# NVIDIA/audio-flamingo

Measured on AMD Instinct MI355X. Metric: audio-sec/s + decoder tokens/s, AF3-7B bf16 train, higher is better.
Workload: dtype bf16; 1 GPU; AF3 (AF-Whisper 32L + Qwen2.5-7B 28L, MLP projector) bf16 train step fwd+bwd+AdamW, 30 s clips, S=1024; micro_batch_per_gpu=8, global_batch=8, seq_len=1024, parallelism=dp1, activation_checkpointing=False

## Files before the change

### audio-flamingo_amd/csrc/gemm.hip

```cpp
#include "gemm_common.h"
#include <vector>
#include <mutex>

namespace {

constexpr int BM = 128, BN = 128, BK = 64;
constexpr int ROWB = BK * 2;
constexpr int STAGE_BYTES = (BM + BN) * ROWB;
constexpr int NSTAGE = 2;

__global__ __launch_bounds__(256, 2) void gemm_nt_bf16_k128(GemmArgs p) {
    extern __shared__ __attribute__((aligned(16))) char smem[];
    const int tid = threadIdx.x;
    const int lane = tid & 63;
    const int wave = __builtin_amdgcn_readfirstlane(tid >> 6);
    const int wm = wave >> 1, wn = wave & 1;
    const int hi = lane >> 5, l31 = lane & 31;

    int tm, tn;
    gemm_tile_of_block(p, tm, tn);
    const int m0 = tm * BM, n0 = tn * BN;

    const bf16* a_src[4];
    const bf16* b_src[4];
// ... 82 lines not shown
    const int lane = threadIdx.x & 63, wave = threadIdx.x >> 6;
    const int n0 = (blockIdx.x * 4 + wave) * R;
    if (n0 >= p.N) return;
    const int kb_all = (p.K + 511) >> 9;
    const int kb0 = (int)((int64_t)kb_all * blockIdx.y / p.splits), kb1 = (int)((int64_t)kb_all * (blockIdx.y + 1) / p.splits);
    float acc[R][MB];
#pragma unroll
    for (int r = 0; r < R; ++r)
#pragma unroll
        for (int m = 0; m < MB; ++m) acc[r][m] = 0.f;
    const bf16* wrow[R];
#pragma unroll
    for (int r = 0; r < R; ++r) wrow[r] = p.B + (int64_t)min(n0 + r, p.N - 1) * p.ldb;
    for (int kb = kb0; kb < kb1; ++kb) {
        const int k = (kb << 9) + lane * 8;
        if (k < p.K) {
            bf16x8 wv[R], xv[MB];
#pragma unroll
            for (int r = 0; r < R; ++r) wv[r] = __builtin_nontemporal_load((const bf16x8*)(wrow[r] + k));
#pragma unroll
            for (int m = 0; m < MB; ++m) xv[m] = *(const bf16x8*)(p.A + (int64_t)min(m, p.M - 1) * p.lda + k);
#pragma unroll
            for (int r = 0; r < R; ++r)
#pragma unroll
                for (int m = 0; m < MB; ++m)
#pragma unroll
                    for (int e = 0; e < 4; ++e) {
                        const bf16x2 a = {wv[r][2 * e], wv[r][2 * e + 1]}, b = {xv[m][2 * e], xv[m][2 * e + 1]};
                        acc[r][m] = __builtin_amdgcn_fdot2_f32_bf16(a, b, acc[r][m], false);
                    }
        }
    }
    constexpr int V = R * MB;
    static_assert((V & (V - 1)) == 0 && V <= 64, "R*MB must be a power of two <= 64");
    float* v = &acc[0][0];
    int n = V;
#pragma unroll
    for (int sft = 5; sft >= 0; --sft) {
        const int st = 1 << sft;
        const bool up = (lane >> sft) & 1;
        if (n > 1) {
            const int h = n >> 1;
#pragma unroll
            for (int i = 0; i < V / 2; ++i)
                if (i < h) {
                    const float lo = v[i], hi_ = v[i + h];
                    v[i] = (up ? hi_ : lo) + __shfl_xor(up ? lo : hi_, st, 64);
                }
            n = h;
        } else {
            v[0] += __shfl_xor(v[0], st, 64);
        }
    }
    constexpr int LOGV = V == 64 ? 6 : V == 32 ? 5 : V == 16 ? 4 : V == 8 ? 3 : V == 4 ? 2 : V == 2 ? 1 : 0;
    const int idx = lane >> (6 - LOGV);
    const int r = idx / MB, m = idx % MB;
    if ((lane & ((64 >> LOGV) - 1)) == 0 && n0 + r < p.N && m < p.M) p.ws[((int64_t)blockIdx.y * p.M + m) * p.N + n0 + r] = v[0];
}

__global__ __launch_bounds__(256) void gemm_splitk_reduce_kernel(GemmArgs p) {
    const int n4 = p.N >> 2;
    const int64_t total = (int64_t)p.M * n4;
    for (int64_t t = (int64_t)blockIdx.x * blockDim.x + threadIdx.x; t < total; t += (int64_t)gridDim.x * blockDim.x) {
        const int m = (int)(t / n4), n = (int)(t % n4) * 4;
        const float* src = p.ws + (int64_t)m * p.N + n;
        f32x4 acc = *(const f32x4*)src;
        for (int sp = 1; sp < p.splits; ++sp) {
            const f32x4 x = *(const f32x4*)(src + (int64_t)sp * p.M * p.N);
#pragma unroll
            for (int e = 0; e < 4; ++e) acc[e] += x[e];
        }
        float v[4] = {acc[0], acc[1], acc[2], acc[3]};
        gemm_epilogue_store4(p, m, n, v);
    }
}

struct ProfState {
    std::mutex mu;
    bool on = false;
    std::vector<hipEvent_t> pool;
    size_t used = 0;
    double flops = 0.0;
    int64_t launches = 0;
    struct Rec { int M, N, K, variant; };
    std::vector<Rec> recs;
};
ProfState g_prof;
int g_variant = 0;
[[maybe_unused]] int g_256_impl = 2;
int g_gm = 0;
int g_wide = 1;
int g_mfma = 0;

constexpr int mfma_shapes(int form) { return form == 0 ? AFK_MFMA_SHAPES_NT : form == 1 ? AFK_MFMA_SHAPES_NN : AFK_MFMA_SHAPES_TN; }
constexpr int AFK_MFMA_RULE_NT = 16, AFK_MFMA_RULE_NN = 32, AFK_MFMA_RULE_TN = 32;
int gemm_mfma_of(int form) {
    static const int env = [] {
        const char* e = getenv("AFK_GEMM_MFMA");
        return (e && e[0] >= '0' && e[0] <= '2' && !e[1]) ? e[0] - '0' : 0;
    }();
    const int sel = g_mfma ? g_mfma : env;
    if (sel == 1) return 32;
    if (sel == 2) return 16;
    return form == 0 ? AFK_MFMA_RULE_NT : form == 1 ? AFK_MFMA_RULE_NN : AFK_MFMA_RULE_TN;
}

hipEvent_t prof_next_event() {
    if (g_prof.used == g_prof.pool.size()) {
        hipEvent_t e;
        hipEventCreate(&e);
        g_prof.pool.push_back(e);
    }
    return g_prof.pool[g_prof.used++];
}

}

extern "C" int afk_gemm_set_variant(int v) {
    const int gm = (v >> 8) & 255, base = v & 15;
#ifdef AFK_PROBES
    AFK_REQUIRE(base >= 0 && base <= 14, "afk_gemm_set_variant: 14 = persistent tile loop with the next tile's prologue issued ahead of the epilogue stores (round-4 probe), 13 = 256x256 ping-pong as a persistent tile loop, 0 auto, 1 = 128x128, 2 = 256x256 8-wave ping-pong, 3 = 256x256 4-wave (4, 5: its timing probes), 6 = 256x256 8-wave free-running BK=64 (7, 8, 9: probes), 10 = 8-wave free-running BK=32 ring-10 (11: probe)");
#else
    AFK_REQUIRE(base >= 0 && base <= 2, "afk_gemm_set_variant: variant %d is a probe / rejected schedule; this libafk.so was built without -DAFK_PROBES (make PROBES=1)", base);
    AFK_REQUIRE((gm & 0xc0) == 0, "afk_gemm_set_variant: gm bits 6 / 7 are timing probes (wrong results); this libafk.so was built without -DAFK_PROBES");
#endif
    g_gm = gm;
    g_wide = (v & 16) ? 0 : 1;
    g_variant = base;
    return AFK_OK;
}

extern "C" int afk_gemm_set_mfma(int v) {
    AFK_REQUIRE(v >= 0 && v <= 2, "afk_gemm_set_mfma: %d (0 = dispatch rule, 1 = 32x32x16, 2 = 16x16x32)", v);
    constexpr int any = AFK_MFMA_SHAPES_NT | AFK_MFMA_SHAPES_NN | AFK_MFMA_SHAPES_TN;
    AFK_REQUIRE(v == 0 || (any >> (v - 1)) & 1, "afk_gemm_set_mfma: no 256x256 kernel of this libafk.so carries the %s shape; build with make PROBES=1",
                v == 1 ? "32x32x16" : "16x16x32");
    g_mfma = v;
    return AFK_OK;
}
extern "C" int afk_gemm_mfma_shapes(int form) { return form >= 0 && form <= 2 ? mfma_shapes(form) : 0; }

extern "C" int afk_prof_enable(int on) {
    std::lock_guard<std::mutex> lk(g_prof.mu);
    g_prof.on = on != 0;
    return AFK_OK;
}

extern "C" int afk_prof_reset(void) {
    std::lock_guard<std::mutex> lk(g_prof.mu);
    g_prof.used = 0;
    g_prof.flops = 0.0;
    g_prof.launches = 0;
    g_prof.recs.clear();
    return AFK_OK;
}

extern "C" int afk_prof_collect(double* total_ms, double* total_flops, int64_t* launches) {
    std::lock_guard<std::mutex> lk(g_prof.mu);
    double ms = 0.0;
    for (size_t i = 0; i + 1 < g_prof.used; i += 2) {
        if (hipEventSynchronize(g_prof.pool[i + 1]) != hipSuccess)
            return afk_set_error(AFK_ERR_LAUNCH, "afk_prof_collect: event sync failed");
        float t = 0.f;
        if (hipEventElapsedTime(&t, g_prof.pool[i], g_prof.pool[i + 1]) != hipSuccess)
            return afk_set_error(AFK_ERR_LAUNCH, "afk_prof_collect: elapsed failed");
        ms += t;
    }
    if (total_ms) *total_ms = ms;
    if (total_flops) *total_flops = g_prof.flops;
    if (launches) *launches = g_prof.launches;
    return AFK_OK;
}

struct RopeEpi { const void *cos_t, *sin_t; const int* pos; int S, cols; const void *cos_lanes, *sin_lanes; };

static int gemm_impl(int trans_a, int trans_b, const void* A, int64_t lda, const void* B, int64_t ldb, void* C, int64_t ldc,
                     int M, int N, int K, const void* bias, const void* residual, int64_t ldr,
                     int res_mod, void* preact_out, float alpha, int flags, void* stream, int splits = 1, void* workspace = nullptr,
                     const RopeEpi* rope = nullptr) {
    AFK_REQUIRE(splits >= 1 && splits <= 64 && (splits == 1 || workspace), "afk_gemm_*_splitk: 1..64 splits, workspace required");
    AFK_REQUIRE(((flags & AFK_GEMM_ROPE) != 0) == (rope != nullptr), "afk_gemm: AFK_GEMM_ROPE belongs to afk_gemm_nt_bf16_rope");
    AFK_REQUIRE(splits == 1 || splits <= (K + BK - 1) / BK, "afk_gemm_*_splitk: more splits than K tiles");
    const bool gemv = workspace != nullptr && M <= AFK_GEMV_MAX_M && !trans_a && !trans_b;
    AFK_REQUIRE(!gemv || splits <= (K + 511) / 512, "afk_gemm_nt_bf16_splitk: M <= 16 streams K in blocks of 512: at most ceil(K/512) splits");
    AFK_REQUIRE(A && B && C, "afk_gemm_nt_bf16: null operand");
    AFK_REQUIRE(M > 0 && N > 0 && K > 0, "afk_gemm_nt_bf16: bad shape %d %d %d", M, N, K);
    AFK_REQUIRE(!trans_a || trans_b, "afk_gemm_bf16: A^T with k-contiguous B is not implemented (NT, NN, TN are)");
    AFK_REQUIRE(trans_a || K % BK == 0, "afk_gemm_nt_bf16: K=%d must be a multiple of %d (pad the operand)", K, BK);
    AFK_REQUIRE(!trans_b || (N % 8 == 0 && N >= 8), "afk_gemm_bf16: N=%d must be a multiple of 8 for a reduction-major B", N);
    AFK_REQUIRE(!trans_a || (M % 8 == 0 && M >= 8), "afk_gemm_bf16: M=%d must be a multiple of 8 for a reduction-major A", M);
    AFK_REQUIRE(N % 4 == 0, "afk_gemm_nt_bf16: N=%d must be a multiple of 4", N);
    AFK_REQUIRE(lda % 8 == 0 && ldb % 8 == 0 && ldc % 4 == 0, "afk_gemm_nt_bf16: leading dims must keep 16-B (A,B) / 8-B (C) alignment");
    AFK_REQUIRE(!(flags & AFK_GEMM_BIAS) || bias, "afk_gemm_nt_bf16: BIAS flag without bias");
    AFK_REQUIRE(!(flags & AFK_GEMM_RESIDUAL) || (residual && ldr % 4 == 0), "afk_gemm_nt_bf16: RESIDUAL flag without residual");
    AFK_REQUIRE(!(flags & AFK_GEMM_SWIGLU_FWD) || (flags == AFK_GEMM_SWIGLU_FWD && !trans_a && !trans_b && preact_out && N % 256 == 0 && splits == 1 &&
                                                     ldc % 8 == 0 && (uintptr_t)C % 16 == 0 && (uintptr_t)preact_out % 16 == 0),
                "afk_gemm_nt_bf16: SWIGLU_FWD needs the NT form, preact_out, N = 2I with I %% 128 == 0 and no other flag");
    AFK_REQUIRE(!(flags & AFK_GEMM_SWIGLU_BWD) || (residual && ldr % 4 == 0 && ldc >= 2 * (int64_t)N && flags == AFK_GEMM_SWIGLU_BWD && splits == 1),
                "afk_gemm: SWIGLU_BWD needs the gate|up tensor as `residual`, a [M, 2N] output and no other epilogue flag");
    AFK_REQUIRE(((uintptr_t)A % 16 == 0) && ((uintptr_t)B % 16 == 0) && ((uintptr_t)C % 8 == 0), "afk_gemm_nt_bf16: misaligned pointer");
    GemmArgs p;
    p.A = (const bf16*)A;
    p.B = (const bf16*)B;
    p.C = C;
    p.C2 = preact_out;
    p.bias = (const bf16*)bias;
    p.R = (const bf16*)residual;
    p.lda = lda;
    p.ldb = ldb;
    p.ldc = ldc;
    p.ldr = ldr;
    p.M = M;
    p.N = N;
    p.K = K;
    p.flags = flags;
    p.res_mod = res_mod;
    p.alpha = alpha;
    p.gm = g_gm;
    p.splits = splits;
    p.ws = (float*)workspace;
    p.rope_cos = rope ? (const bf16*)rope->cos_t : nullptr;
    p.rope_sin = rope ? (const bf16*)rope->sin_t : nullptr;
    p.rope_pos = rope ? rope->pos : nullptr;
    p.rope_S = rope ? rope->S : 1;
    p.rope_cols = rope ? rope->cols : 0;
    const bool lanes_ok = rope && rope->cos_lanes && rope->sin_lanes && !rope->pos && rope->S % 32 == 0;
    p.rope_cos_lanes = lanes_ok ? (const bf16*)rope->cos_lanes : nullptr;
    p.rope_sin_lanes = lanes_ok ? (const bf16*)rope->sin_lanes : nullptr;
    {
        const bool f32 = (flags & AFK_GEMM_OUT_F32) != 0;
        bool w = N % 8 == 0 && ldc % 8 == 0 && (uintptr_t)C % (f32 ? 32 : 16) == 0;
        if (flags & AFK_GEMM_BIAS) w = w && (uintptr_t)bias % 16 == 0;
        if (flags & (AFK_GEMM_RESIDUAL | AFK_GEMM_SWIGLU_BWD)) w = w && ldr % 8 == 0 && (uintptr_t)residual % 16 == 0;
        if (preact_out) w = w && (uintptr_t)preact_out % 16 == 0;
        p.wide = w && g_wide ? 1 : 0;
    }
    const int64_t tiles256 = afk_cdiv(M, 256) * afk_cdiv(N, 256);
    const bool use256 = !gemv && (trans_b || (flags & AFK_GEMM_SWIGLU_FWD) || (splits == 1 && (g_variant >= 2 || (g_variant == 0 && tiles256 >= 192))));
    if (rope && (!use256 || !p.wide || trans_a || trans_b || splits != 1))
        return afk_set_error(AFK_ERR_UNSUPPORTED, "afk_gemm_nt_bf16_rope: needs the 256 x 256 NT kernel (>= 192 tiles) in its 16-byte epilogue form; use "
                                                  "afk_gemm_nt_bf16 + afk_rope_inplace for this shape");
#ifdef AFK_PROBES
    static const int env_impl = [] {
        const char* e = getenv("AFK_GEMM256");
        return (e && e[0] == 'p' && e[1] == 'e') ? 13 : (e && e[0] == 'p') ? 2 : (e && e[0] == 'w') ? 3 : (e && e[0] == 'f') ? 10 : 0;
    }();
    const int impl256 = (flags & (AFK_GEMM_SWIGLU_FWD | AFK_GEMM_ROPE)) ? 2 : g_variant >= 2 ? g_variant : (env_impl ? env_impl : g_256_impl);
    const bool w4 = use256 && !trans_b && impl256 >= 3 && impl256 <= 9;
    const bool f8 = use256 && !trans_b && impl256 >= 10 && impl256 <= 12;
    const bool persist = use256 && !trans_b && impl256 == 13;
    const bool persist_q = use256 && !trans_b && impl256 == 14;
#endif
    if ((flags & AFK_GEMM_SWIGLU_FWD) && !p.wide)
        return afk_set_error(AFK_ERR_UNSUPPORTED, "afk_gemm_nt_bf16: SWIGLU_FWD needs the 16-byte epilogue form (aligned C / preact_out, ldc %% 8 == 0, "
                                                  "afk_gemm_set_variant bit 4 clear)");
    p.ntm = (int)afk_cdiv(M, use256 ? 256 : BM);
    p.ntn = (int)afk_cdiv(N, use256 ? 256 : BN);
    static bool attr_set = false;
    if (!attr_set) {
        hipFuncSetAttribute((const void*)gemm_nt_bf16_k128, hipFuncAttributeMaxDynamicSharedMemorySize, NSTAGE * STAGE_BYTES);
        attr_set = true;
    }
    hipStream_t st = (hipStream_t)stream;
    const int64_t nwg = (int64_t)p.ntm * p.ntn;
    AFK_REQUIRE(nwg < (1ll << 31), "afk_gemm_nt_bf16: grid too large");
    hipEvent_t e0 = nullptr, e1 = nullptr;
    bool prof = false;
    {
        std::lock_guard<std::mutex> lk(g_prof.mu);
        prof = g_prof.on;
        if (prof) {
            e0 = prof_next_event();
            e1 = prof_next_event();
            g_prof.flops += 2.0 * (double)M * (double)N * (double)K;
            g_prof.launches += 1;
            g_prof.recs.push_back({M, N, K, trans_b ? (trans_a ? 4 : 3) : (use256 ? 2 : 1)});
        }
    }
    afk_count(gemv ? AFK_CNT_GEMV : trans_b ? (trans_a ? AFK_CNT_GEMM_TN256 : AFK_CNT_GEMM_NN256) : use256 ? AFK_CNT_GEMM_NT256 : AFK_CNT_GEMM_NT128);
    if (splits > 1) afk_count(AFK_CNT_GEMM_SPLITK);
    if (prof) hipEventRecord(e0, st);
    if (gemv) {
        const dim3 grid((unsigned)afk_cdiv(N, 32), (unsigned)splits);
#define AFK_GEMV(MB_, R_) hipLaunchKernelGGL((gemv_nt_bf16_kernel<MB_, R_>), grid, dim3(256), 0, st, p)
        AFK_GEMV(1, 8);
#undef AFK_GEMV
        int g = (int)afk_cdiv((int64_t)M * (N / 4), 256);
        if (g > 2048) g = 2048;
        hipLaunchKernelGGL(gemm_splitk_reduce_kernel, dim3(g), dim3(256), 0, st, p);
    } else if (trans_b) {
        if (int e = afk_launch_gemm256t(p, trans_a, gemm_mfma_of(trans_a ? 2 : 1), st)) return e;
        if (splits > 1) {
            int g = (int)afk_cdiv((int64_t)M * (N / 4), 256);
            if (g > 2048) g = 2048;
            hipLaunchKernelGGL(gemm_splitk_reduce_kernel, dim3(g), dim3(256), 0, st, p);
        }
    } else if (use256) {
#ifdef AFK_PROBES
        if (int e = persist_q ? afk_launch_gemm256q(p, st) : persist ? afk_launch_gemm256p(p, st) : f8 ? afk_launch_gemm256f8(p, impl256 - 10, st) : w4 ? afk_launch_gemm256w4(p, impl256 - 3, st) : afk_launch_gemm256(p, gemm_mfma_of(0), st)) return e;
#else
        if (int e = afk_launch_gemm256(p, gemm_mfma_of(0), st)) return e;
#endif
    } else {
        hipLaunchKernelGGL(gemm_nt_bf16_k128, dim3((unsigned)nwg, (unsigned)splits), dim3(256), NSTAGE * STAGE_BYTES, st, p);
        if (splits > 1) {
            int g = (int)afk_cdiv((int64_t)M * (N / 4), 256);
            if (g > 2048) g = 2048;
            hipLaunchKernelGGL(gemm_splitk_reduce_kernel, dim3(g), dim3(256), 0, st, p);
        }
    }
    if (prof) hipEventRecord(e1, st);
    AFK_LAUNCH_CHECK("afk_gemm_nt_bf16");
    return AFK_OK;
}

extern "C" int afk_gemm_nt_bf16(const void* A, int64_t lda, const void* B, int64_t ldb, void* C, int64_t ldc,
                                int M, int N, int K, const void* bias, const void* residual, int64_t ldr,
                                int res_mod, void* preact_out, float alpha, int flags, void* stream) {
    return gemm_impl(0, 0, A, lda, B, ldb, C, ldc, M, N, K, bias, residual, ldr, res_mod, preact_out, alpha, flags, stream);
}

extern "C" int afk_gemm_nt_bf16_rope(const void* A, int64_t lda, const void* B, int64_t ldb, void* C, int64_t ldc, int M, int N, int K, const void* bias,
                                     const void* cos_t, const void* sin_t, const int* pos, int S, int rope_cols, const void* cos_lanes, const void* sin_lanes,
                                     void* stream) {
    AFK_REQUIRE(cos_t && sin_t && (uintptr_t)cos_t % 16 == 0 && (uintptr_t)sin_t % 16 == 0, "afk_gemm_nt_bf16_rope: cos / sin tables (16-byte aligned) are required");
    AFK_REQUIRE(N % 256 == 0 && rope_cols >= 0 && rope_cols <= N && rope_cols % 256 == 0 && S > 0,
                "afk_gemm_nt_bf16_rope: N and rope_cols must be multiples of 256 (two 128-column heads per tile), S > 0");
    AFK_REQUIRE((cos_lanes == nullptr) == (sin_lanes == nullptr) && (!cos_lanes || ((uintptr_t)cos_lanes % 16 == 0 && (uintptr_t)sin_lanes % 16 == 0)),
                "afk_gemm_nt_bf16_rope: the lane-major tables come as a 16-byte aligned pair");
    const RopeEpi r = {cos_t, sin_t, pos, S, rope_cols, cos_lanes, sin_lanes};
    return gemm_impl(0, 0, A, lda, B, ldb, C, ldc, M, N, K, bias, nullptr, 0, 0, nullptr, 1.f, AFK_GEMM_ROPE | (bias ? AFK_GEMM_BIAS : 0), stream, 1, nullptr, &r);
}

extern "C" int afk_gemm_nt_bf16_splitk(const void* A, int64_t lda, const void* B, int64_t ldb, void* C, int64_t ldc, int M, int N, int K,
                                       const void* bias, const void* residual, int64_t ldr, int res_mod, void* preact_out, float alpha,
                                       int flags, int splits, void* workspace, void* stream) {
    return gemm_impl(0, 0, A, lda, B, ldb, C, ldc, M, N, K, bias, residual, ldr, res_mod, preact_out, alpha, flags, stream, splits, workspace);
}

extern "C" int afk_gemv_partials(const void* A, int64_t lda, const void* B, int64_t ldb, int M, int N, int K, int splits, float* workspace,
                                 void* stream) {
    AFK_REQUIRE(A && B && workspace && M >= 1 && M <= AFK_GEMV_MAX_M && N > 0 && K > 0 && K % 8 == 0 && lda % 8 == 0 && ldb % 8 == 0,
                "afk_gemv_partials: bad args (M <= %d, K %% 8 == 0)", AFK_GEMV_MAX_M);
    AFK_REQUIRE(splits >= 1 && splits <= (K + 511) / 512 && splits <= 64, "afk_gemv_partials: 1 <= splits <= ceil(K / 512)");
    GemmArgs p = {};
    p.A = (const bf16*)A; p.B = (const bf16*)B; p.lda = lda; p.ldb = ldb; p.M = M; p.N = N; p.K = K; p.splits = splits; p.ws = workspace;
    const dim3 grid((unsigned)afk_cdiv(N, 32), (unsigned)splits);
    hipStream_t st = (hipStream_t)stream;
    hipLaunchKernelGGL((gemv_nt_bf16_kernel<1, 8>), grid, dim3(256), 0, st, p);
    AFK_LAUNCH_CHECK("afk_gemv_partials");
    return AFK_OK;
}

extern "C" int afk_gemm_bf16_splitk(int trans_a, int trans_b, const void* A, int64_t lda, const void* B, int64_t ldb, void* C, int64_t ldc,
                                    int M, int N, int K, const void* bias, const void* residual, int64_t ldr, int res_mod, void* preact_out,
                                    float alpha, int flags, int splits, void* workspace, void* stream) {
    return gemm_impl(trans_a, trans_b, A, lda, B, ldb, C, ldc, M, N, K, bias, residual, ldr, res_mod, preact_out, alpha, flags, stream, splits,
                     workspace);
}

extern "C" int afk_gemm_bf16(int trans_a, int trans_b, const void* A, int64_t lda, const void* B, int64_t ldb, void* C,
                             int64_t ldc, int M, int N, int K, const void* bias, const void* residual, int64_t ldr,
                             int res_mod, void* preact_out, float alpha, int flags, void* stream) {
    return gemm_impl(trans_a, trans_b, A, lda, B, ldb, C, ldc, M, N, K, bias, residual, ldr, res_mod, preact_out, alpha, flags, stream);
}

extern "C" int afk_prof_dump(const char* host_path) {
    std::lock_guard<std::mutex> lk(g_prof.mu);
    FILE* f = fopen(host_path, "w");
    if (!f) return afk_set_error(AFK_ERR_ARG, "afk_prof_dump: cannot open %s", host_path);
    fprintf(f, "M,N,K,variant,ms\n");
    for (size_t i = 0; i < g_prof.recs.size() && 2 * i + 1 < g_prof.used; ++i) {
        float ms = 0.f;
        hipEventSynchronize(g_prof.pool[2 * i + 1]);
        hipEventElapsedTime(&ms, g_prof.pool[2 * i], g_prof.pool[2 * i + 1]);
        fprintf(f, "%d,%d,%d,%d,%.6f\n", g_prof.recs[i].M, g_prof.recs[i].N, g_prof.recs[i].K, g_prof.recs[i].variant, ms);
    }
    fclose(f);
    return AFK_OK;
}
```

### audio-flamingo_amd/csrc/gemm256t.hip

```cpp
#include "gemm_common.h"

namespace {

constexpr int BK = 64;
constexpr int OP_BYTES = 32768;
constexpr int BUF_BYTES = 2 * OP_BYTES;
constexpr int LDS_BYTES = 2 * BUF_BYTES;
constexpr int TROW = 512;

typedef __attribute__((address_space(3))) bf16x4 lds_bf16x4;

#define AFK_VMCNT(n) asm volatile("s_waitcnt vmcnt(" #n ")" ::: "memory")
#define AFK_LGKMCNT0() asm volatile("s_waitcnt lgkmcnt(0)" ::: "memory")
#define AFK_BARRIER()                         \
    do {                                      \
        __builtin_amdgcn_sched_barrier(0);    \
        __builtin_amdgcn_s_barrier();         \
        __builtin_amdgcn_sched_barrier(0);    \
    } while (0)
#define AFK_DMA_PTR(SRCPTR, DSTPTR)                                                                       \
    do {                                                                                                  \
        __builtin_amdgcn_sched_barrier(0);                                                                \
        __builtin_amdgcn_global_load_lds((gbl_void*)(SRCPTR), (lds_void*)(DSTPTR), 16, 0, 0);             \
        __builtin_amdgcn_sched_barrier(0);                                                                \
    } while (0)

__device__ __forceinline__ int tswz(int r) { return ((r & 3) << 2) | ((r >> 2) & 3); }

template <int MF>
__device__ __forceinline__ int tr_off(int tile, int pc, int lane) {
    const int g = lane >> 4, i = lane & 15;
    const int chunk = MF == 16 ? 2 * tile + ((i & 3) >> 1) : 4 * tile + 2 * (g & 1) + ((i & 3) >> 1);
    const int r = (MF == 16 ? 8 * g : 8 * (g >> 1)) + (i >> 2) + 4 * pc;
    return r * TROW + ((chunk ^ tswz(r)) << 4) + 8 * (i & 1);
}
template <int MF, int S>
__device__ __forceinline__ bf16x8 tr_frag(uint32_t buf, int off0, int off1) {
    return afk_lds_tr_frag<S * (48 - MF) * TROW>(buf + off0, buf + off1);
}

struct TSrc {
    const bf16* base;
    int krow;
};
__device__ __forceinline__ TSrc tsrc(const bf16* mat, int unit, int col0, int ncols, int lane) {
    const int krow = 2 * unit + (lane >> 5);
    const int pos = lane & 31;
    const int chunk = pos ^ tswz(krow);
    const int col = min(col0 + chunk * 8, ncols - 8);
    TSrc s;
    s.base = mat + col;
    s.krow = krow;
    return s;
}

template <bool AT, int EPI, int MF>
__global__ __launch_bounds__(512, 1) void gemm_xt_bf16_k256(GemmArgs p) {
    extern __shared__ __attribute__((aligned(16))) char smem[];
    const int tid = threadIdx.x;
    const int lane = tid & 63;
    const int wave = __builtin_amdgcn_readfirstlane(tid >> 6);
    const int wm = wave >> 2, wn = wave & 3;
    const int hi = lane >> 5, l31 = lane & 31;

    int tm, tn;
    gemm_tile_of_block(p, tm, tn);
    const int m0 = tm * 256, n0 = tn * 256;
    int KL = p.K;
    const bf16* Abase = p.A;
    const bf16* Bbase = p.B;
    if (p.splits > 1) {
        const int tall = (p.K + BK - 1) / BK;
        const int t0 = (int)((int64_t)tall * blockIdx.y / p.splits), t1 = (int)((int64_t)tall * (blockIdx.y + 1) / p.splits);
        const int kbeg = t0 * BK;
        KL = min(p.K, t1 * BK) - kbeg;
        Abase += AT ? (int64_t)kbeg * p.lda : (int64_t)kbeg;
        Bbase += (int64_t)kbeg * p.ldb;
    }
    const int T = (KL + BK - 1) / BK;
    constexpr int NX = AT ? 4 : 6, NY = AT ? 4 : 2;

    const bf16* an_src[NX + NY];
    TSrc tr_src[NX + NY];
    int64_t tr_ld[NX + NY];
    int dst[NX + NY];
#pragma unroll
    for (int j = 0; j < NX + NY; ++j) {
        const bool isx = j < NX;
        const int jj = isx ? j : j - NX;
        an_src[j] = nullptr;
        tr_src[j].base = nullptr;
        tr_src[j].krow = 0;
        tr_ld[j] = 0;
        if (AT) {
            const bool isA = jj < 2;
            const int unit = (isx ? 0 : 16) + wave + 8 * (jj & 1);
            tr_src[j] = isA ? tsrc(Abase, unit, m0, p.M, lane) : tsrc(Bbase, unit, n0, p.N, lane);
            tr_ld[j] = isA ? p.lda : p.ldb;
            dst[j] = (isA ? 0 : OP_BYTES) + unit * 1024;
        } else if (isx && jj < 4) {
            const int unit = wave + 8 * jj;
            tr_src[j] = tsrc(Bbase, unit, n0, p.N, lane);
            tr_ld[j] = p.ldb;
            dst[j] = OP_BYTES + unit * 1024;
        } else {
            const int k = wave + 8 * (isx ? jj - 4 : jj);
            const int unit = isx ? (k < 8 ? k : k + 8) : (k < 8 ? 8 + k : 16 + k);
            const int rl = unit * 8 + (lane >> 3);
            const int chunk = (lane & 7) ^ ((rl >> 1) & 7);
            const int r = min(m0 + rl, p.M - 1);
            an_src[j] = Abase + (int64_t)r * p.lda + chunk * 8;
            dst[j] = unit * 1024;
        }
    }
    const bf16* tbase[NX + NY];
#pragma unroll
    for (int j = 0; j < NX + NY; ++j) tbase[j] = (AT || j < 4) ? tr_src[j].base + (int64_t)tr_src[j].krow * tr_ld[j] : nullptr;
    GemmAcc<MF> acc;
    acc.zero();

    const bool ragged = (KL % BK) != 0;
  auto pipeline = [&](auto rag_) {
    constexpr bool RAG = decltype(rag_)::value;
    auto src_of = [&](int j, int t) -> const bf16* {
        const bool tr = AT || j < 4;
        if (tr) {
            if constexpr (RAG) {
                const int row = min(t * BK + tr_src[j].krow, KL - 1);
                return tr_src[j].base + (int64_t)row * tr_ld[j];
            } else {
                return tbase[j] + (int64_t)t * BK * tr_ld[j];
            }
        }
        return an_src[j] + (int64_t)t * BK;
    };
    auto issue = [&](int j, int t_src, int parity) { AFK_DMA_PTR(src_of(j, t_src), smem + parity * BUF_BYTES + dst[j]); };

    constexpr int NH = MF == 16 ? 2 : 1;
    int tob[2][NH][2], toa[4][NH][2];
#pragma unroll
    for (int j = 0; j < 2; ++j)
#pragma unroll
        for (int h = 0; h < NH; ++h)
#pragma unroll
            for (int pc = 0; pc < 2; ++pc) tob[j][h][pc] = OP_BYTES + tr_off<MF>((wn * 2 + j) * NH + h, pc, lane);
#pragma unroll
    for (int i = 0; i < 4; ++i)
#pragma unroll
        for (int h = 0; h < NH; ++h)
#pragma unroll
            for (int pc = 0; pc < 2; ++pc) toa[i][h][pc] = AT ? tr_off<MF>((wm * 4 + i) * NH + h, pc, lane) : 0;
    auto tr_read = [&](uint32_t lbuf, const int (&to)[NH][2], auto x_, auto ks0_) {
        constexpr int x = decltype(x_)::value, ks0 = decltype(ks0_)::value;
        if constexpr (MF == 32) return tr_frag<MF, ks0 + x>(lbuf, to[0][0], to[0][1]);
        else if constexpr (AT) return tr_frag<MF, ks0>(lbuf, to[x][0], to[x][1]);
        else return tr_frag<MF, (x & 1)>(lbuf, to[x >> 1][0], to[x >> 1][1]);
    };
    int koffb[4];
#pragma unroll
    for (int x = 0; x < 4; ++x) koffb[x] = gemm_frag_rowoff<MF>(x) * 128 + gemm_frag_koff<MF>(x, lane);
    const int a_row0 = (wm * 128 + gemm_frag_row<MF>(lane)) * 128;

#pragma unroll
    for (int j = 0; j < NX; ++j) issue(j, 0, 0);
#pragma unroll
    for (int j = 0; j < NY; ++j) issue(NX + j, 0, 0);
    {
        const int t1 = min(1, T - 1);
#pragma unroll
        for (int j = 0; j < NX; ++j) issue(j, t1, 1);
    }
    if (AT) AFK_VMCNT(8); else AFK_VMCNT(8);
    AFK_BARRIER();
    if (wm == 1) AFK_BARRIER();

    bf16x8 bf[2][4], af[AT ? 4 : 2][AT ? 2 : 4];
    const uint32_t lds0 = afk_lds_addr(smem);
    for (int t = 0; t < T; ++t) {
        const char* buf = smem + (t & 1) * BUF_BYTES;
        const uint32_t lbuf = lds0 + (t & 1) * BUF_BYTES;
        const int t1 = min(t + 1, T - 1), t2 = min(t + 2, T - 1);
        const int e1 = (t + 1) & 1, e2 = t & 1;
        if constexpr (!AT) {
#pragma unroll
            for (int j = 0; j < 2; ++j)
                afk_static_for<4>([&](auto x_) { bf[j][decltype(x_)::value] = tr_read(lbuf, tob[j], x_, std::integral_constant<int, 0>{}); });
#pragma unroll
            for (int i = 0; i < 2; ++i)
#pragma unroll
                for (int s = 0; s < 4; ++s) af[i][s] = *(const bf16x8*)(buf + a_row0 + i * 32 * 128 + koffb[s]);
            AFK_LGKMCNT0();
            AFK_VMCNT(6);
            AFK_BARRIER();
            __builtin_amdgcn_s_setprio(1);
            afk_static_for<4>([&](auto g_) {
                constexpr int g = decltype(g_)::value;
                if constexpr (MF == 32) {
#pragma unroll
                    for (int i = 0; i < 2; ++i)
#pragma unroll
                        for (int j = 0; j < 2; ++j) acc.mma(i, j, bf[j][g], af[i][g]);
                } else {
                    constexpr int s = g >> 1, i = g & 1;
#pragma unroll
                    for (int ih = 0; ih < 2; ++ih)
#pragma unroll
                        for (int jt = 0; jt < 4; ++jt) acc.mma(2 * i + ih, jt, bf[jt >> 1][2 * (jt & 1) + s], af[i][2 * ih + s]);
                }
                if constexpr (g < 2) issue(NX + g, t1, e1);
            });
            __builtin_amdgcn_s_setprio(0);
            AFK_VMCNT(8);
            AFK_BARRIER();
#pragma unroll
            for (int i = 0; i < 2; ++i)
#pragma unroll
                for (int s = 0; s < 4; ++s) af[i][s] = *(const bf16x8*)(buf + a_row0 + (i + 2) * 32 * 128 + koffb[s]);
            AFK_LGKMCNT0();
            AFK_VMCNT(2);
            AFK_BARRIER();
            __builtin_amdgcn_s_setprio(1);
            afk_static_for<8>([&](auto q_) {
                constexpr int piece = decltype(q_)::value;
                if constexpr (MF == 32) {
                    constexpr int s = piece >> 1, i = piece & 1;
                    acc.mma(2 + i, 0, bf[0][s], af[i][s]);
                    acc.mma(2 + i, 1, bf[1][s], af[i][s]);
                } else {
                    constexpr int s = piece >> 2, i = (piece >> 1) & 1, ih = piece & 1;
#pragma unroll
                    for (int jt = 0; jt < 4; ++jt) acc.mma(2 * (2 + i) + ih, jt, bf[jt >> 1][2 * (jt & 1) + s], af[i][2 * ih + s]);
                }
                if constexpr (piece < 6) issue(piece, t2, e2);
            });
            __builtin_amdgcn_s_setprio(0);
            AFK_VMCNT(8);
            AFK_BARRIER();
        } else {
            const int kvalid = KL - t * BK;
#pragma unroll
            for (int ph = 0; ph < 2; ++ph) {
                afk_static_for<2>([&](auto x_) {
                    constexpr int x = decltype(x_)::value;
                    constexpr int KS = MF == 16 ? 1 : 2;
                    if (ph == 0) {
#pragma unroll
                        for (int j = 0; j < 2; ++j) bf[j][x] = tr_read(lbuf, tob[j], x_, std::integral_constant<int, 0>{});
#pragma unroll
                        for (int i = 0; i < 4; ++i) af[i][x] = tr_read(lbuf, toa[i], x_, std::integral_constant<int, 0>{});
                    } else {
#pragma unroll
                        for (int j = 0; j < 2; ++j) bf[j][x] = tr_read(lbuf, tob[j], x_, std::integral_constant<int, KS>{});
#pragma unroll
                        for (int i = 0; i < 4; ++i) af[i][x] = tr_read(lbuf, toa[i], x_, std::integral_constant<int, KS>{});
                    }
                });
                AFK_LGKMCNT0();
                if (RAG && kvalid < BK) {
#pragma unroll
                    for (int s = 0; s < 2; ++s)
#pragma unroll
                        for (int e = 0; e < 8; ++e) {
                            const bool dead = (MF == 16 ? 32 * ph + 8 * (lane >> 4) : 16 * (2 * ph + s) + 8 * hi) + e >= kvalid;
#pragma unroll
                            for (int i = 0; i < 4; ++i)
                                if (dead) af[i][s][e] = (bf16)0.f;
                        }
                }
                AFK_VMCNT(4);
                AFK_BARRIER();
                __builtin_amdgcn_s_setprio(1);
                afk_static_for<8>([&](auto q_) {
                    constexpr int piece = decltype(q_)::value;
                    if constexpr (MF == 32) {
                        constexpr int s = piece >> 2, i = piece & 3;
                        acc.mma(i, 0, bf[0][s], af[i][s]);
                        acc.mma(i, 1, bf[1][s], af[i][s]);
                    } else {
                        constexpr int i = piece >> 1, ih = piece & 1;
#pragma unroll
                        for (int jt = 0; jt < 4; ++jt) acc.mma(2 * i + ih, jt, bf[jt >> 1][jt & 1], af[i][ih]);
                    }
                    if constexpr ((piece & 1) == 0) {
                        if (ph == 0) issue(NX + (piece >> 1), t1, e1);
                        else issue(piece >> 1, t2, e2);
                    }
                });
                __builtin_amdgcn_s_setprio(0);
                AFK_VMCNT(8);
                AFK_BARRIER();
            }
        }
    }
    AFK_VMCNT(0);
    if (wm == 0) AFK_BARRIER();
  };
    if (ragged) pipeline(std::true_type{});
    else pipeline(std::false_type{});

#pragma unroll
    for (int i = 0; i < 4; ++i)
#pragma unroll
        for (int j = 0; j < 2; ++j) gemm_store_block32<EPI, MF>(p, m0 + wm * 128 + i * 32, n0 + wn * 64 + j * 32, lane, acc.block(i, j));
}

}

#define AFK_EPI_LIST(X) X(0) X(AFK_GEMM_ACCUM) X(-2) X(-1)

template <bool AT, int MF>
static int launch_gemm256t(const GemmArgs& p, hipStream_t st) {
    static bool attr_set = false;
    if (!attr_set) {
#define AFK_SET(F)                                                                                                                              \
    if (hipFuncSetAttribute((const void*)gemm_xt_bf16_k256<AT, (F), MF>, hipFuncAttributeMaxDynamicSharedMemorySize, LDS_BYTES) != hipSuccess) \
        return afk_set_error(AFK_ERR_LAUNCH, "gemm256t: cannot reserve %d bytes of LDS", LDS_BYTES);
        AFK_EPI_LIST(AFK_SET)
#undef AFK_SET
        attr_set = true;
    }
    const int64_t nwg = (int64_t)p.ntm * p.ntn;
    const unsigned ns = (unsigned)(p.splits > 1 ? p.splits : 1);
    const int f = p.splits > 1 ? -2 : (p.wide ? p.flags : -1);
    const dim3 grid((unsigned)nwg, ns);
    switch (f) {
#define AFK_CASE(F)                                                                                        \
    case (F):                                                                                              \
        if ((F) == -1) afk_count(AFK_CNT_GEMM_GENERIC);                                                    \
        hipLaunchKernelGGL((gemm_xt_bf16_k256<AT, (F), MF>), grid, dim3(512), LDS_BYTES, st, p);           \
        break;
        AFK_EPI_LIST(AFK_CASE)
#undef AFK_CASE
        default:
            afk_count(AFK_CNT_GEMM_GENERIC);
            hipLaunchKernelGGL((gemm_xt_bf16_k256<AT, -1, MF>), grid, dim3(512), LDS_BYTES, st, p);
    }
    return AFK_OK;
}

int afk_launch_gemm256t(const GemmArgs& p, int trans_a, int mf, hipStream_t st) {
    if (trans_a) {
        if constexpr ((AFK_MFMA_SHAPES_TN & 2) != 0)
            if (mf == 16) return launch_gemm256t<true, 16>(p, st);
        if constexpr ((AFK_MFMA_SHAPES_TN & 1) != 0)
            if (mf == 32) return launch_gemm256t<true, 32>(p, st);
    } else {
        if constexpr ((AFK_MFMA_SHAPES_NN & 2) != 0)
            if (mf == 16) return launch_gemm256t<false, 16>(p, st);
        if constexpr ((AFK_MFMA_SHAPES_NN & 1) != 0)
            if (mf == 32) return launch_gemm256t<false, 32>(p, st);
    }
    return afk_set_error(AFK_ERR_UNSUPPORTED, "gemm256t: the %s MFMA shape of the %s kernel is built under make PROBES=1 only", mf == 16 ? "16x16x32" : "32x32x16",
                         trans_a ? "TN" : "NN");
}
```

### include/afk.h

```cpp
#ifndef AFK_H
#define AFK_H
#include <stdint.h>
#ifdef __cplusplus
extern "C" {
#endif

int afk_version(void);
const char* afk_last_error(void);
const char* afk_build_id(void);
int afk_has_probes(void);

#define AFK_CNT_GEMM_NT128 0
#define AFK_CNT_GEMM_NT256 1
#define AFK_CNT_GEMM_NN256 2
#define AFK_CNT_GEMM_TN256 3
#define AFK_CNT_GEMM_SPLITK 4
#define AFK_CNT_GEMV 5
#define AFK_CNT_ATTN2_FWD_D64 6
#define AFK_CNT_ATTN2_FWD_D128 7
#define AFK_CNT_ATTN2_BWD_D64 8
#define AFK_CNT_ATTN2_BWD_D128 9
#define AFK_CNT_GQA_REDUCE 10
#define AFK_CNT_XATTN_FWD 11
#define AFK_CNT_XATTN_BWD 12
#define AFK_CNT_ATTN1_FWD 13
#define AFK_CNT_ATTN1_BWD 14
#define AFK_CNT_GEMM_GENERIC 15
#define AFK_CNT_MAX 16
int afk_kernel_counts(int64_t* host_out, int n);
int afk_kernel_counts_reset(void);

int afk_prof_enable(int on);
int afk_prof_reset(void);
int afk_prof_collect(double* host_total_ms, double* host_total_flops, int64_t* host_launches);
int afk_prof_dump(const char* host_path);

int afk_gemm_set_variant(int variant);
int afk_gemm_set_mfma(int v);
int afk_gemm_mfma_shapes(int form);
#define AFK_GEMM_BIAS 1
#define AFK_GEMM_GELU 2
#define AFK_GEMM_RESIDUAL 4
#define AFK_GEMM_OUT_F32 8
#define AFK_GEMM_ACCUM 16
#define AFK_GEMM_SWIGLU_BWD 32
#define AFK_GEMM_ROPE 128
#define AFK_GEMM_SWIGLU_FWD 64
int afk_gemm_nt_bf16(const void* A, int64_t lda, const void* B, int64_t ldb, void* C, int64_t ldc,
                     int M, int N, int K, const void* bias, const void* residual, int64_t ldr,
                     int res_mod, void* preact_out, float alpha, int flags, void* stream);
int afk_gemm_bf16(int trans_a, int trans_b, const void* A, int64_t lda, const void* B, int64_t ldb, void* C,
                  int64_t ldc, int M, int N, int K, const void* bias, const void* residual, int64_t ldr,
                  int res_mod, void* preact_out, float alpha, int flags, void* stream);
int afk_gemm_nt_bf16_rope(const void* A, int64_t lda, const void* B, int64_t ldb, void* C, int64_t ldc, int M, int N, int K, const void* bias,
                          const void* cos_t, const void* sin_t, const int* pos, int S, int rope_cols, const void* cos_lanes, const void* sin_lanes, void* stream);
int afk_gemm_nt_bf16_splitk(const void* A, int64_t lda, const void* B, int64_t ldb, void* C, int64_t ldc, int M, int N, int K,
                            const void* bias, const void* residual, int64_t ldr, int res_mod, void* preact_out, float alpha,
                            int flags, int splits, void* workspace, void* stream);
int afk_gemm_bf16_splitk(int trans_a, int trans_b, const void* A, int64_t lda, const void* B, int64_t ldb, void* C, int64_t ldc,
                         int M, int N, int K, const void* bias, const void* residual, int64_t ldr, int res_mod, void* preact_out,
                         float alpha, int flags, int splits, void* workspace, void* stream);


int afk_norm_bwd_blocks(int64_t rows);
int afk_layernorm_fwd(const void* x, const void* w, const void* b, void* y, float* mean, float* rstd,
                      int64_t rows, int D, float eps, void* stream);
int afk_layernorm_bwd(const void* x, const void* w, const void* dy, const float* mean, const float* rstd,
                      void* dx, const void* dx_add, void* dw, void* db, int accumulate, float* workspace,
                      int64_t rows, int D, void* stream);
int afk_rmsnorm_fwd(const void* x, const void* w, void* y, float* rstd, int64_t rows, int D, float eps, void* stream);
int afk_gelu_bwd_colsum_parts(int64_t rows);
int afk_gelu_bwd_colsum(const void* dy, const void* pre, void* dx, int64_t rows, int C, void* colsum, int colsum_accumulate, float* workspace, void* stream);
int afk_layernorm_bwd_colsum(const void* x, const void* w, const void* dy, const float* mean, const float* rstd, void* dx, const void* dx_add, void* dw, void* db,
                             int accumulate, void* colsum, int colsum_accumulate, float* workspace, int64_t rows, int D, void* stream);
int afk_rmsnorm_bwd(const void* x, const void* w, const void* dy, const float* rstd, void* dx, const void* dx_add,
                    void* dw, int accumulate, float* workspace, int64_t rows, int D, void* stream);

int afk_transpose_bf16(const void* in, void* out, int R, int C, int Rpad, int64_t ld_in, int64_t ld_out, int nb1,
                       int nb2, int64_t bs1_in, int64_t bs2_in, int64_t bs1_out, int64_t bs2_out, int max_blocks, void* stream);
int afk_gelu_fwd(const void* x, void* y, int64_t n, void* stream);
int afk_gelu_bwd(const void* dy, const void* pre, void* dx, int64_t n, void* stream);
int afk_silu_mul_fwd(const void* gu, void* h, int64_t rows, int I, void* stream);
int afk_silu_mul_bwd(const void* gu, const void* dh, void* dgu, int64_t rows, int I, void* stream);
int afk_rope_inplace(void* buf, const void* cos_t, const void* sin_t, const int* pos, int64_t rows, int S, int ld,
                     int nheads, int D, int backward, void* stream);
int afk_add_bf16(const void* a, const void* b, void* out, int64_t n, void* stream);
int afk_cast_f32_bf16(const float* in, void* out, int64_t n, void* stream);
int afk_scale_add_bf16(const void* x, void* y, int64_t n, const float* scale_dev, int accumulate, void* stream);
int afk_rowsum_bf16(const void* in, int64_t ld, int C, void* out, int rows, int accumulate, void* stream);

int afk_colsum_slices(int64_t rows);
int afk_colsum_bf16(const void* in, int64_t ld, int64_t rows, int cols, void* out, int accumulate, float* workspace, void* stream);
int afk_colsum_bf16_fused(const void* in, int64_t ld, int64_t rows, int cols, void* out, int accumulate, float* workspace, int* counters, void* stream);

int afk_relu_fwd(const void* x, void* y, int64_t n, void* stream);
int afk_relu_bwd(const void* dy, const void* y, void* dx, int64_t n, void* stream);
int afk_gate_fwd(const void* x, const void* h, const void* alpha, int alpha_is_vector, const int* gate, void* y, int64_t rows,
                 int D, void* stream);
int afk_gate_bwd(const void* dy, const void* h, const void* alpha, int alpha_is_vector, const int* gate, void* dh,
                 float* fws, void* dalpha, int accumulate, int64_t rows, int D, void* stream);

int afk_im2col_conv1(const void* x, int x_is_f32, void* col, int W, int C, int T, void* stream);
int afk_im2col_conv2(const void* h, void* col, int W, int Tin, int Tout, int C, void* stream);
int afk_col2im_conv2(const void* dcol, void* dh, int W, int Tin, int Tout, int C, void* stream);
int afk_conv_weight_permute(const void* in, void* out, int Co, int Ci, int dir, int accumulate, void* stream);
int afk_avgpool2_fwd(const void* x, void* y, int64_t out_rows, int C, void* stream);
int afk_avgpool2_bwd(const void* dy, void* dx, int64_t out_rows, int C, void* stream);

int afk_placeholder_scan(const int64_t* ids, int64_t n, int64_t audio_id, int* src, int* n_audio, void* stream);
int afk_embed_scatter_fwd(const int64_t* ids, const int* src, const void* embed, const void* audio, void* out,
                          int64_t n, int H, void* stream);
int afk_embed_scatter_bwd(const int64_t* ids, const int* src, const void* dout, void* d_embed, void* d_audio,
                          const int* perm, int64_t n, int H, void* stream);

int afk_attn_fwd(const void* Q, int64_t q_bs, int64_t q_hs, int64_t q_rs, const void* K, int64_t k_bs, int64_t k_hs,
                 int64_t k_rs, const void* Vt, void* O, int64_t o_bs, int64_t o_hs, int64_t o_rs, float* LSE,
                 const int* kv_len, int B, int Hq, int Hkv, int S, int Spad, int D, float scale, int causal, void* stream);
int afk_attn_delta(const void* O, int64_t o_bs, int64_t o_hs, int64_t o_rs, const void* dO, int64_t do_bs,
                   int64_t do_hs, int64_t do_rs, float* delta, int B, int H, int S, int D, void* stream);
int afk_attn_bwd(const void* Q, int64_t q_bs, int64_t q_hs, int64_t q_rs, const void* K, int64_t k_bs, int64_t k_hs,
// ... 208 lines not shown
```

Before: 639.1 audio-s/s.

## Widen 256-tile NT dispatch for deep-K shapes and split ragged-K tail in transposed GEMM

The NT dispatch rule now picks the 256x256 kernel for shapes with at least 168 tiles when K is at least 3584, not only at 192 or more tiles. A public afk_gemm_nt_tile query exposes that choice. In the transposed 256 kernel the ragged-K path is restructured: all but the last few K tiles run the non-ragged fast path, and only the tail runs the clamped and masked version. Rematerialised lane values, precomputed per-lane limits and accumulator pinning are added to limit register pressure, at the cost of more code and extra setup. The profiler records also gain flags and splits fields.

```diff
diff --git a/audio-flamingo_amd/csrc/gemm.hip b/audio-flamingo_amd/csrc/gemm.hip
--- a/audio-flamingo_amd/csrc/gemm.hip
+++ b/audio-flamingo_amd/csrc/gemm.hip
@@ -188,7 +188,7 @@
     size_t used = 0;
     double flops = 0.0;
     int64_t launches = 0;
-    struct Rec { int M, N, K, variant; };
+    struct Rec { int M, N, K, variant, flags, splits; };
     std::vector<Rec> recs;
 };
 ProfState g_prof;
@@ -211,6 +211,14 @@
     return form == 0 ? AFK_MFMA_RULE_NT : form == 1 ? AFK_MFMA_RULE_NN : AFK_MFMA_RULE_TN;
 }
 
+constexpr int64_t NT256_FULL_TILES = 192;
+constexpr int64_t NT256_FEW_TILES = 168;
+constexpr int64_t NT256_FEW_MIN_K = 3584;
+bool gemm_nt_wants_256(int64_t M, int64_t N, int64_t K) {
+    const int64_t tiles256 = afk_cdiv(M, 256) * afk_cdiv(N, 256);
+    return tiles256 >= NT256_FULL_TILES || (tiles256 >= NT256_FEW_TILES && K >= NT256_FEW_MIN_K);
+}
+
 hipEvent_t prof_next_event() {
     if (g_prof.used == g_prof.pool.size()) {
         hipEvent_t e;
@@ -235,6 +243,8 @@
     g_variant = base;
     return AFK_OK;
 }
+
+extern "C" int afk_gemm_nt_tile(int M, int N, int K) { return M > 0 && N > 0 && K > 0 && gemm_nt_wants_256(M, N, K) ? 256 : 128; }
 
 extern "C" int afk_gemm_set_mfma(int v) {
     AFK_REQUIRE(v >= 0 && v <= 2, "afk_gemm_set_mfma: %d (0 = dispatch rule, 1 = 32x32x16, 2 = 16x16x32)", v);
@@ -341,10 +351,9 @@
         if (preact_out) w = w && (uintptr_t)preact_out % 16 == 0;
         p.wide = w && g_wide ? 1 : 0;
     }
-    const int64_t tiles256 = afk_cdiv(M, 256) * afk_cdiv(N, 256);
-    const bool use256 = !gemv && (trans_b || (flags & AFK_GEMM_SWIGLU_FWD) || (splits == 1 && (g_variant >= 2 || (g_variant == 0 && tiles256 >= 192))));
+    const bool use256 = !gemv && (trans_b || (flags & AFK_GEMM_SWIGLU_FWD) || (splits == 1 && (g_variant >= 2 || (g_variant == 0 && gemm_nt_wants_256(M, N, K)))));
     if (rope && (!use256 || !p.wide || trans_a || trans_b || splits != 1))
-        return afk_set_error(AFK_ERR_UNSUPPORTED, "afk_gemm_nt_bf16_rope: needs the 256 x 256 NT kernel (>= 192 tiles) in its 16-byte epilogue form; use "
+        return afk_set_error(AFK_ERR_UNSUPPORTED, "afk_gemm_nt_bf16_rope: needs the 256 x 256 NT kernel (afk_gemm_nt_tile) in its 16-byte epilogue form; use "
                                                   "afk_gemm_nt_bf16 + afk_rope_inplace for this shape");
 #ifdef AFK_PROBES
     static const int env_impl = [] {
@@ -380,7 +389,7 @@
             e1 = prof_next_event();
             g_prof.flops += 2.0 * (double)M * (double)N * (double)K;
             g_prof.launches += 1;
-            g_prof.recs.push_back({M, N, K, trans_b ? (trans_a ? 4 : 3) : (use256 ? 2 : 1)});
+            g_prof.recs.push_back({M, N, K, trans_b ? (trans_a ? 4 : 3) : (use256 ? 2 : 1), flags, splits});
         }
     }
     afk_count(gemv ? AFK_CNT_GEMV : trans_b ? (trans_a ? AFK_CNT_GEMM_TN256 : AFK_CNT_GEMM_NN256) : use256 ? AFK_CNT_GEMM_NT256 : AFK_CNT_GEMM_NT128);
@@ -475,12 +484,12 @@
     std::lock_guard<std::mutex> lk(g_prof.mu);
     FILE* f = fopen(host_path, "w");
     if (!f) return afk_set_error(AFK_ERR_ARG, "afk_prof_dump: cannot open %s", host_path);
-    fprintf(f, "M,N,K,variant,ms\n");
+    fprintf(f, "M,N,K,variant,ms,flags,splits\n");
     for (size_t i = 0; i < g_prof.recs.size() && 2 * i + 1 < g_prof.used; ++i) {
         float ms = 0.f;
         hipEventSynchronize(g_prof.pool[2 * i + 1]);
         hipEventElapsedTime(&ms, g_prof.pool[2 * i], g_prof.pool[2 * i + 1]);
-        fprintf(f, "%d,%d,%d,%d,%.6f\n", g_prof.recs[i].M, g_prof.recs[i].N, g_prof.recs[i].K, g_prof.recs[i].variant, ms);
+        fprintf(f, "%d,%d,%d,%d,%.6f,%d,%d\n", g_prof.recs[i].M, g_prof.recs[i].N, g_prof.recs[i].K, g_prof.recs[i].variant, ms, g_prof.recs[i].flags, g_prof.recs[i].splits);
     }
     fclose(f);
     return AFK_OK;
diff --git a/audio-flamingo_amd/csrc/gemm256t.hip b/audio-flamingo_amd/csrc/gemm256t.hip
--- a/audio-flamingo_amd/csrc/gemm256t.hip
+++ b/audio-flamingo_amd/csrc/gemm256t.hip
@@ -52,6 +52,19 @@
     s.base = mat + col;
     s.krow = krow;
     return s;
+}
+
+__device__ __forceinline__ void acc_pin(GemmAcc<32>& a) {
+#pragma unroll
+    for (int i = 0; i < 4; ++i)
+#pragma unroll
+        for (int j = 0; j < 2; ++j) asm volatile("" : "+v"(a.v[i][j]));
+}
+__device__ __forceinline__ void acc_pin(GemmAcc<16>& a) {
+#pragma unroll
+    for (int i = 0; i < 8; ++i)
+#pragma unroll
+        for (int j = 0; j < 4; ++j) asm volatile("" : "+v"(a.v[i][j]));
 }
 
 template <bool AT, int EPI, int MF>
@@ -114,42 +127,49 @@
         }
     }
     const bf16* tbase[NX + NY];
-#pragma unroll
-    for (int j = 0; j < NX + NY; ++j) tbase[j] = (AT || j < 4) ? tr_src[j].base + (int64_t)tr_src[j].krow * tr_ld[j] : nullptr;
+    int tkrow[NX + NY];
+#pragma unroll
+    for (int j = 0; j < NX + NY; ++j) {
+        tbase[j] = (AT || j < 4) ? tr_src[j].base + (int64_t)tr_src[j].krow * tr_ld[j] : nullptr;
+        tkrow[j] = tr_src[j].krow;
+    }
     GemmAcc<MF> acc;
     acc.zero();
 
-    const bool ragged = (KL % BK) != 0;
-  auto pipeline = [&](auto rag_) {
-    constexpr bool RAG = decltype(rag_)::value;
-    auto src_of = [&](int j, int t) -> const bf16* {
+    const bool ragged = AT && (KL % BK) != 0;
+    int tnow = 0;
+    auto src_of = [&](auto rag_, int j, int t) -> const bf16* {
+        constexpr bool RAG = decltype(rag_)::value;
         const bool tr = AT || j < 4;
         if (tr) {
             if constexpr (RAG) {
-                const int row = min(t * BK + tr_src[j].krow, KL - 1);
-                return tr_src[j].base + (int64_t)row * tr_ld[j];
+                const int row = min(t * BK + tkrow[j], KL - 1);
+                return tbase[j] + (int64_t)(row - tkrow[j] - tnow * BK) * tr_ld[j];
             } else {
                 return tbase[j] + (int64_t)t * BK * tr_ld[j];
             }
         }
         return an_src[j] + (int64_t)t * BK;
     };
-    auto issue = [&](int j, int t_src, int parity) { AFK_DMA_PTR(src_of(j, t_src), smem + parity * BUF_BYTES + dst[j]); };
+    auto issue = [&](auto rag_, int j, int t_src, int parity) { AFK_DMA_PTR(src_of(rag_, j, t_src), smem + parity * BUF_BYTES + dst[j]); };
 
     constexpr int NH = MF == 16 ? 2 : 1;
     int tob[2][NH][2], toa[4][NH][2];
-#pragma unroll
-    for (int j = 0; j < 2; ++j)
-#pragma unroll
-        for (int h = 0; h < NH; ++h)
-#pragma unroll
-            for (int pc = 0; pc < 2; ++pc) tob[j][h][pc] = OP_BYTES + tr_off<MF>((wn * 2 + j) * NH + h, pc, lane);
-#pragma unroll
-    for (int i = 0; i < 4; ++i)
-#pragma unroll
-        for (int h = 0; h < NH; ++h)
-#pragma unroll
-            for (int pc = 0; pc < 2; ++pc) toa[i][h][pc] = AT ? tr_off<MF>((wm * 4 + i) * NH + h, pc, lane) : 0;
+    auto frag_offsets = [&](int ln) {
+#pragma unroll
+        for (int j = 0; j < 2; ++j)
+#pragma unroll
+            for (int h = 0; h < NH; ++h)
+#pragma unroll
+                for (int pc = 0; pc < 2; ++pc) tob[j][h][pc] = OP_BYTES + tr_off<MF>((wn * 2 + j) * NH + h, pc, ln);
+#pragma unroll
+        for (int i = 0; i < 4; ++i)
+#pragma unroll
+            for (int h = 0; h < NH; ++h)
+#pragma unroll
+                for (int pc = 0; pc < 2; ++pc) toa[i][h][pc] = AT ? tr_off<MF>((wm * 4 + i) * NH + h, pc, ln) : 0;
+    };
+    frag_offsets(lane);
     auto tr_read = [&](uint32_t lbuf, const int (&to)[NH][2], auto x_, auto ks0_) {
         constexpr int x = decltype(x_)::value, ks0 = decltype(ks0_)::value;
         if constexpr (MF == 32) return tr_frag<MF, ks0 + x>(lbuf, to[0][0], to[0][1]);
@@ -162,13 +182,13 @@
     const int a_row0 = (wm * 128 + gemm_frag_row<MF>(lane)) * 128;
 
 #pragma unroll
-    for (int j = 0; j < NX; ++j) issue(j, 0, 0);
-#pragma unroll
-    for (int j = 0; j < NY; ++j) issue(NX + j, 0, 0);
+    for (int j = 0; j < NX; ++j) issue(std::bool_constant<AT>{}, j, 0, 0);
+#pragma unroll
+    for (int j = 0; j < NY; ++j) issue(std::bool_constant<AT>{}, NX + j, 0, 0);
     {
         const int t1 = min(1, T - 1);
 #pragma unroll
-        for (int j = 0; j < NX; ++j) issue(j, t1, 1);
+        for (int j = 0; j < NX; ++j) issue(std::bool_constant<AT>{}, j, t1, 1);
     }
     if (AT) AFK_VMCNT(8); else AFK_VMCNT(8);
     AFK_BARRIER();
@@ -176,7 +196,8 @@
 
     bf16x8 bf[2][4], af[AT ? 4 : 2][AT ? 2 : 4];
     const uint32_t lds0 = afk_lds_addr(smem);
-    for (int t = 0; t < T; ++t) {
+    auto tile = [&](auto rag_, int t) {
+        constexpr bool RAG = decltype(rag_)::value;
         const char* buf = smem + (t & 1) * BUF_BYTES;
         const uint32_t lbuf = lds0 + (t & 1) * BUF_BYTES;
         const int t1 = min(t + 1, T - 1), t2 = min(t + 2, T - 1);
@@ -207,7 +228,7 @@
 #pragma unroll
                         for (int jt = 0; jt < 4; ++jt) acc.mma(2 * i + ih, jt, bf[jt >> 1][2 * (jt & 1) + s], af[i][2 * ih + s]);
                 }
-                if constexpr (g < 2) issue(NX + g, t1, e1);
+                if constexpr (g < 2) issue(rag_, NX + g, t1, e1);
             });
             __builtin_amdgcn_s_setprio(0);
             AFK_VMCNT(8);
@@ -231,13 +252,14 @@
 #pragma unroll
                     for (int jt = 0; jt < 4; ++jt) acc.mma(2 * (2 + i) + ih, jt, bf[jt >> 1][2 * (jt & 1) + s], af[i][2 * ih + s]);
                 }
-                if constexpr (piece < 6) issue(piece, t2, e2);
+                if constexpr (piece < 6) issue(rag_, piece, t2, e2);
             });
             __builtin_amdgcn_s_setprio(0);
             AFK_VMCNT(8);
             AFK_BARRIER();
         } else {
             const int kvalid = KL - t * BK;
+            const int klimit = kvalid - (MF == 16 ? 8 * (lane >> 4) : 8 * hi);
 #pragma unroll
             for (int ph = 0; ph < 2; ++ph) {
                 afk_static_for<2>([&](auto x_) {
@@ -261,7 +283,7 @@
                     for (int s = 0; s < 2; ++s)
 #pragma unroll
                         for (int e = 0; e < 8; ++e) {
-                            const bool dead = (MF == 16 ? 32 * ph + 8 * (lane >> 4) : 16 * (2 * ph + s) + 8 * hi) + e >= kvalid;
+                            const bool dead = (MF == 16 ? 32 * ph : 16 * (2 * ph + s)) + e >= klimit;
 #pragma unroll
                             for (int i = 0; i < 4; ++i)
                                 if (dead) af[i][s][e] = (bf16)0.f;
@@ -282,8 +304,8 @@
                         for (int jt = 0; jt < 4; ++jt) acc.mma(2 * i + ih, jt, bf[jt >> 1][jt & 1], af[i][ih]);
                     }
                     if constexpr ((piece & 1) == 0) {
-                        if (ph == 0) issue(NX + (piece >> 1), t1, e1);
-                        else issue(piece >> 1, t2, e2);
+                        if (ph == 0) issue(rag_, NX + (piece >> 1), t1, e1);
+                        else issue(rag_, piece >> 1, t2, e2);
                     }
                 });
                 __builtin_amdgcn_s_setprio(0);
@@ -291,12 +313,24 @@
                 AFK_BARRIER();
             }
         }
-    }
+    };
+    const int Ts = ragged ? max(T - 3, 0) : T;
+    for (int t = 0; t < Ts; ++t) tile(std::false_type{}, t);
+    if constexpr (AT) {
+        int lane_late = lane;
+        asm volatile("" : "+v"(lane_late));
+#pragma unroll
+        for (int j = 0; j < NX + NY; ++j) {
+            tkrow[j] = 2 * ((j < NX ? 0 : 16) + wave + 8 * (j & 1)) + (lane_late >> 5);
+            tbase[j] += (int64_t)Ts * BK * tr_ld[j];
+        }
+        tnow = Ts;
+        frag_offsets(lane_late);
+    }
+    for (int t = Ts; t < T; ++t) tile(std::true_type{}, t);
     AFK_VMCNT(0);
     if (wm == 0) AFK_BARRIER();
-  };
-    if (ragged) pipeline(std::true_type{});
-    else pipeline(std::false_type{});
+    acc_pin(acc);
 
 #pragma unroll
     for (int i = 0; i < 4; ++i)
diff --git a/include/afk.h b/include/afk.h
--- a/include/afk.h
+++ b/include/afk.h
@@ -36,6 +36,7 @@
 int afk_prof_dump(const char* host_path);
 
 int afk_gemm_set_variant(int variant);
+int afk_gemm_nt_tile(int M, int N, int K);
 int afk_gemm_set_mfma(int v);
 int afk_gemm_mfma_shapes(int form);
 #define AFK_GEMM_BIAS 1
```

After: 641.0 audio-s/s, median of 6. No clear change (+0.3%).
